# xyang9527/dro-sfm

Measured on AMD Instinct MI355X. Metric: training images/sec (KITTI 192x640 mf self-sup), higher is better.
Workload: dtype f32; 1 GPU; KITTI 192x640 mf self-sup (configs[1]); model=DepthPoseNet it8-seq4-inter-out, global_batch=2, per_gpu_batch=2, ref_frames=2, parallelism=dp1, optimizer=Adam lr 2e-4, execution=hipgraph, update_blocks=depth block + pose block (side stream, with both context encoders), encoder_3x3_s1=hip, encoder_strided=hip, exchange=none (world 1)

## Files before the change

dro-sfm_amd/csrc/conv.hip:

```cpp
#include <hip/hip_runtime.h>

#include <algorithm>
#include <cstddef>
#include <cstdio>
#include <cstdlib>
#include <cstring>
#include <map>
#include <mutex>
#include <string>
#include <type_traits>

#include "conv_common.hpp"
#include "dro_common.hpp"

namespace dro {


template <int BM, int MODE, int ACT, int EPI>
__global__ __launch_bounds__(256) void igemm_kernel(IgArgs a) {
  constexpr int WM = BM / 32;
  constexpr int KSTEPS = (WM == 2) ? 16 : 8;
  __shared__ float Ws[2][kBK][BM + 1];
  __shared__ float Xs[2][kBK][kBN];
  const int cb1 = a.cbase[1], cb2 = a.cbase[2], cb3 = a.cbase[3];
  const int H = a.g.H, W = a.g.W, KW = a.g.KW, PH = a.g.PH, PW = a.g.PW;
  const int Hsrc = a.Hs, Wsrc = a.Ws, sh = a.sshift;
  const unsigned HWs = (unsigned)Hsrc * (unsigned)Wsrc;
  const int Cin = a.g.Cin, Cout = a.g.Cout, rows = a.rows, kch = a.kch, K = a.K;
// ... 1025 lines not shown
  static constexpr int T = KH * KW;
  static constexpr bool TAPSPLIT = T == 9 && TG == 1;
  static constexpr int TPW = TAPSPLIT ? 5 : (TG == 3 ? 3 : T);
  static constexpr int TH = HaloShape<32, KH, KW>::TH, TW = 64 / TH;
  static constexpr int HWd = TW + KW - 1;
  static constexpr int HALO = (TH + KH - 1) * HWd;
  static constexpr int HPAD = HALO | 1;
  static constexpr int NJ = (HALO + 63) / 64;
  static constexpr int BC = 64, GPAD = 65;
  static constexpr int STAGE = 64 * GPAD + BC * HPAD;
  static constexpr int RED = TAPSPLIT ? 0 : 4 * 16 * 64;
  static constexpr int LDS = 2 * STAGE > RED ? 2 * STAGE : RED;
  static_assert(NJ <= 2 && TW % 2 == 0, "halo shape");
};

template <int KH, int KW, int GACT, bool MULTI, int TG>
__global__ __launch_bounds__(512) void wgrad2_kernel(typename WgParam<MULTI>::T P) {
  static_assert(TG == 1 || (TG == 3 && KH == 3 && KW == 3), "tap groups: 3x3 rows");
  const IgArgs& a = WgParam<MULTI>::ig(P);
  using S = HaloShapeW2<KH, KW, TG>;
  constexpr int T = S::T, TH = S::TH, TW = S::TW, HWd = S::HWd, HALO = S::HALO, HPAD = S::HPAD;
  constexpr int NJ = S::NJ, BC = S::BC, GPAD = S::GPAD, STAGE = S::STAGE, TPW = S::TPW;
  constexpr bool TAPSPLIT = S::TAPSPLIT;
  constexpr int PH = KH / 2, PW = KW / 2;
  __shared__ float smem[S::LDS];
  const int cb1 = a.cbase[1], cb2 = a.cbase[2], cb3 = a.cbase[3];
  const int H = a.g.H, W = a.g.W, Cin = a.g.Cin, Cout = a.g.Cout;
  const int tid = threadIdx.x, lane = tid & 63;
  const int wave = __builtin_amdgcn_readfirstlane(tid >> 6);
  const int noc = a.otiles * ((Cin + BC - 1) / BC);
  const int nbx = (int)gridDim.x;
  const int lin = xcd_remap((int)(blockIdx.x + blockIdx.y * gridDim.x), (int)(gridDim.x * gridDim.y));
  const int bx = lin % nbx, by = lin / nbx;
  const int tg = TG == 1 ? 0 : bx / noc;
  const int t = bx - tg * noc;
  const int ot = t % a.otiles, ct = t / a.otiles;
  const int o0 = ot * 64, c0 = ct * BC;
  const size_t HW = (size_t)H * W;
  const unsigned HWu = (unsigned)HW;
  int ntiles = a.g.B * a.tiles_img;
  if constexpr (MULTI) ntiles = P.use_tiles * P.nuse;
  const int tbeg = by * a.chunks_per_split;
  const int tend = min(ntiles, tbeg + a.chunks_per_split);
  const bool do_bias = a.gbias && ct == 0 && tg == 0;
  const float galpha = a.galpha;
  float gr[8], yr[GACT ? 8 : 1], xr[8 * NJ], bsum[8];
  unsigned gmask = 0, xmask = 0;
#pragma unroll
  for (int j = 0; j < 8; ++j) bsum[j] = 0.f;
  auto load = [&](int tile) {
    const float* __restrict__ Gp = a.G;
    const float* __restrict__ Yp = a.gy;
    KSlice sbase = kernarg_srcs();
    if constexpr (MULTI) {
      const int u = tile / P.use_tiles;
      tile -= u * P.use_tiles;
      Gp = *(KFPtr)(kernarg_base() + offsetof(WgMulti, uG) + u * sizeof(FPtr));
      if (GACT) Yp = *(KFPtr)(kernarg_base() + offsetof(WgMulti, uy) + u * sizeof(FPtr));
      sbase = (KSlice)(kernarg_base() + offsetof(WgMulti, usrc)) + u * kMaxSrc;
    }
    const int b = tile / a.tiles_img, trem = tile - b * a.tiles_img;
    const int ty0 = (trem / a.tiles_x) * TH, tx0 = (trem % a.tiles_x) * TW;
    const int qy = lane / TW, qx = lane - qy * TW;
    const int oy = ty0 + qy, ox = tx0 + qx;
    const bool pin = oy < H && ox < W;
    const unsigned pix = pin ? (unsigned)(oy * W + ox) : 0u;
    gmask = 0;
#pragma unroll
    for (int j = 0; j < 8; ++j) {
      const int o = o0 + wave * 8 + j;
      const bool ok = pin && o < Cout;
      gmask |= ok ? (1u << j) : 0u;
      const unsigned off = ok ? ((unsigned)b * Cout + o) * HWu + pix : 0u;
      gr[j] = Gp[off];
      if (GACT) yr[j] = Yp[off];
    }
    RowDesc ds[8];
// ... 37 lines not shown
        if (e < HPAD) Xs[(wave + 8 * i) * HPAD + e] = (xmask >> (i * NJ + j)) & 1u ? xr[i * NJ + j] : 0.f;
      }
    }
  };

  const int wo = wave & 1, wc = (wave >> 1) & 1, wg = wave >> 2;
  const int hi = lane >> 5;
  const int tap0 = TAPSPLIT ? wg * 5 : 0;
  const int ntap = TAPSPLIT ? (wg == 0 ? 5 : 4) : T;
  f32x16 acc[TPW];
#pragma unroll
  for (int tp = 0; tp < TPW; ++tp)
#pragma unroll
    for (int r = 0; r < 16; ++r) acc[tp][r] = 0.f;

  if (tbeg < tend) {
    load(tbeg);
    store(0);
  }
  __syncthreads();
  for (int tl = tbeg; tl < tend; ++tl) {
    const int buf = (tl - tbeg) & 1;
    const bool more = tl + 1 < tend;
    if (more) load(tl + 1);
    const float* Gs = smem + buf * STAGE;
    const float* Xs = Gs + 64 * GPAD;
    const float* ga = Gs + hi * GPAD + wo * 32 + (lane & 31);
    const float* xb = Xs + (wc * 32 + (lane & 31)) * HPAD + hi + (TG == 3 ? tg * HWd : 0);
    constexpr int KS = TAPSPLIT ? 32 : 16;
    const int pbase = TAPSPLIT ? 0 : wg * 16;
    auto kloop = [&](auto nt_c, int tbase) __attribute__((always_inline)) {
      constexpr int NT = decltype(nt_c)::value;
      int toff[NT];
#pragma unroll
      for (int k = 0; k < NT; ++k) {
        const int tap = tbase + k;
        toff[k] = (tap / KW) * HWd + (tap % KW);
      }
#pragma unroll 8
// ... 1 lines not shown
        const int pp = 2 * (pbase + s), poff = (pp / TW) * HWd + (pp % TW);
        const float av = ga[pp * GPAD];
#pragma unroll
        for (int k = 0; k < NT; ++k) acc[k] = mfma32(av, xb[poff + toff[k]], acc[k]);
      }
    };
    if constexpr (TAPSPLIT) {
      if (wg == 0) kloop(std::integral_constant<int, 5>{}, 0);
      else kloop(std::integral_constant<int, 4>{}, 5);
    } else {
      kloop(std::integral_constant<int, TPW>{}, 0);
    }
    if (more) store(buf ^ 1);
    __syncthreads();
  }
  float* wpart = a.part + (size_t)by * Cout * Cin * T;
  const int c = c0 + wc * 32 + (lane & 31);
  const size_t tstride = (size_t)Cout * Cin;
  if (TAPSPLIT) {
#pragma unroll
    for (int k = 0; k < TPW; ++k) {
      if (k < ntap) {
#pragma unroll
        for (int r = 0; r < 16; ++r) {
          const int o = o0 + wo * 32 + (r & 3) + 8 * (r >> 2) + 4 * (lane >> 5);
          if (o < Cout && c < Cin) wpart[(tap0 + k) * tstride + (size_t)o * Cin + c] = acc[k][r];
        }
      }
    }
  } else {
    float* red = smem;
// ... 9 lines not shown
#pragma unroll
        for (int r = 0; r < 16; ++r) {
          const int o = o0 + wo * 32 + (r & 3) + 8 * (r >> 2) + 4 * (lane >> 5);
          if (o < Cout && c < Cin)
            wpart[(tg * TPW + tp) * tstride + (size_t)o * Cin + c] = acc[tp][r] + red[(q4 * 16 + r) * 64 + lane];
        }
      }
      __syncthreads();
    }
  }
  if (do_bias) {
#pragma unroll
    for (int j = 0; j < 8; ++j) {
      const float v = wave_sum(bsum[j]);
      const int o = o0 + wave * 8 + j;
      if (lane == 0 && o < Cout) a.bpart[(size_t)by * Cout + o] = v;
    }
  }
}


template <int Q>
__global__ __launch_bounds__(256) void wgrad2_finish_kernel(IgArgs a, int splits) {
  constexpr int EPW = 64 / Q;
  const int Cout = a.g.Cout, Cin = a.g.Cin, T = a.g.KH * a.g.KW;
  const long long oc = (long long)Cout * Cin, total = oc * T;
  const int lane = threadIdx.x & 63, q = lane / EPW, le = lane - q * EPW;
  const int per = (splits + Q - 1) / Q;
  const int s0 = min(splits, q * per), n = min(splits, s0 + per) - s0;
  const long long wstride = (long long)gridDim.x * (blockDim.x / 64) * EPW;
  for (long long eb = ((long long)blockIdx.x * (blockDim.x / 64) + (threadIdx.x >> 6)) * EPW; eb < total;
       eb += wstride) {
    const long long e = eb + le;
    const bool ok = e < total;
    float v = ok ? split_sum(a.part + (size_t)s0 * total + e, (size_t)total, n) : 0.f;
    if (Q >= 4) v += __shfl_xor(v, 2 * EPW);
    if (Q >= 2) {
      const float o = __shfl_xor(v, EPW);
      v = q & 1 ? o + v : v + o;
    }
    if (ok && q == 0) {
      const int tap = (int)(e / oc);
      const long long r = e - (long long)tap * oc;
      const size_t dst = (size_t)r * T + tap;
      a.gweight[dst] = a.wacc ? a.gweight[dst] + v : v;
    }
  }
  if (a.gbias) {
    for (int e = blockIdx.x * blockDim.x + threadIdx.x; e < Cout; e += gridDim.x * blockDim.x) {
      const float bv = split_sum(a.bpart + e, (size_t)Cout, splits);
      a.gbias[e] = a.wacc ? a.gbias[e] + bv : bv;
    }
  }
}

static void launch_wgrad2_finish(const IgArgs& a, int splits, hipStream_t s) {
  const long long total = (long long)a.g.Cout * a.g.Cin * a.g.KH * a.g.KW;
  const int Q = splits >= 32 ? 4 : splits >= 8 ? 2 : 1;
  long long blocks = (total * Q + 255) / 256;
  if (blocks > 4096) blocks = 4096;
  if (Q == 4) hipLaunchKernelGGL(wgrad2_finish_kernel<4>, dim3((unsigned)blocks), dim3(256), 0, s, a, splits);
  else if (Q == 2) hipLaunchKernelGGL(wgrad2_finish_kernel<2>, dim3((unsigned)blocks), dim3(256), 0, s, a, splits);
  else hipLaunchKernelGGL(wgrad2_finish_kernel<1>, dim3((unsigned)blocks), dim3(256), 0, s, a, splits);
}

__global__ __launch_bounds__(256) void wgrad_halo_finish_kernel(IgArgs a, int splits) {
  const int Cout = a.g.Cout;
  const long long total = (long long)Cout * a.g.Cin * a.g.KH * a.g.KW;
// ... 2056 lines not shown
    else { DRO_WHM(3, 3); }
#undef DRO_WHM
  }
  if ((st = launch_status("wgrad_halo_kernel<multi> launch failed"))) return st;
  const long long total = (long long)Cout * Cin * T;
  long long blocks = (total + 255) / 256;
  if (blocks > 2048) blocks = 2048;
  if (v2)
    launch_wgrad2_finish(a, wh.splits, s);
  else
    hipLaunchKernelGGL(wgrad_halo_finish_kernel, dim3((unsigned)blocks), dim3(256), 0, s, a, wh.splits);
  return launch_status("wgrad_halo_finish_kernel launch failed");
}

namespace dro {
__global__ __launch_bounds__(256) void gru_elem_kernel(int stage, int hd, int HW,
                                                       const float* __restrict__ dhn,
                                                       const float* __restrict__ zr,
                                                       const float* __restrict__ q,
                                                       const float* __restrict__ h,
                                                       const float* __restrict__ drh,
                                                       float* __restrict__ dq,
                                                       float* __restrict__ dzr,
                                                       float* __restrict__ dh) {
  const int n = hd * HW;
  const int j = blockIdx.x * 256 + threadIdx.x;
  if (j >= n) return;
  const size_t b = blockIdx.y;
  const size_t i = b * n + j;
  const size_t zi = b * 2 * n + j, ri = zi + n;
// ... 35 lines not shown
```

dro-sfm_amd/hip/_lib.py:

```python
import ctypes
import os

import torch

_HERE = os.path.dirname(os.path.abspath(__file__))
LIB_PATH = os.environ.get("DRO_LIB_PATH") or os.path.normpath(os.path.join(_HERE, "..", "libdro_amd.so"))

_c_float_p = ctypes.c_void_p
_lib = None


def _sig(fn, *argtypes, restype=ctypes.c_int):
    fn.argtypes = list(argtypes)
    fn.restype = restype


def load():
    global _lib
    if _lib is not None:
        return _lib
    if not os.path.exists(LIB_PATH):
        raise RuntimeError(
            f"dro_sfm_amd: native library not found at {LIB_PATH}; build it with "
            "`make -C dro-sfm_amd/csrc` (or __graft_entry__.build()).  There is no CPU fallback.")
# ... 52 lines not shown
    _sig(lib.dro_batchnorm_relu_forward, P, P, P, P, I, I, I, I, F, F, P, P, P, P, P, P, P, Z, S)
    _sig(lib.dro_batchnorm_relu_backward, P, P, P, P, P, P, I, I, I, I, P, P, P, P, P, Z, S)
    _sig(lib.dro_conv2d_workspace_bytes, I, I, I, I, I, I, I, restype=Z)
    _sig(lib.dro_conv2d_plan, I, I, I, I, I, I, I, P)
    _sig(lib.dro_debug_conv_stamps, P)
    _sig(lib.dro_conv_log, I)
    _sig(lib.dro_conv_log_read, ctypes.c_char_p, ctypes.c_longlong, restype=ctypes.c_longlong)
    _sig(lib.dro_weight_split_bytes, I, I, I, I, I, restype=Z)
    _sig(lib.dro_weight_split, P, I, I, I, I, P, P, S)
    _sig(lib.dro_conv2d_forward, P, I, P, P, I, I, I, I, I, I, I, F, P, I, I, P, P, Z, S)
    _sig(lib.dro_convgru_gates_forward, P, I, P, P, I, I, I, I, I, I, P, P, P, P, Z, S)
    _sig(lib.dro_convgru_blend_forward, P, I, P, P, I, I, I, I, I, I, P, P, P, P, I, I, P, P, Z, S)
    _sig(lib.dro_conv2d_backward, P, I, P, I, I, I, I, I, I, I, F, P, P, P, P, P, P, P, P, I, P, P, Z, S)
    _sig(lib.dro_conv2d_weight_grad_multi_workspace_bytes, I, I, I, I, I, I, I, I, restype=Z)
    _sig(lib.dro_conv2d_weight_grad_multi, P, I, I, I, I, I, I, I, I, I, F, P, P, I, P, Z, S)
    _sig(lib.dro_adam_step, P, P, P, P, ctypes.c_longlong, P, P, S)
    _sig(lib.dro_gru_backward_elem, I, I, I, I, I, P, P, P, P, P, P, P, P, S)
    _sig(lib.dro_convgru_candidate_backward, P, I, P, I, I, I, I, I, I, P, P, P, P, P, P, P, P, P, P, Z, S)
    _sig(lib.dro_convgru_gates_backward, P, I, P, I, I, I, I, I, I, P, P, P, P, P, P, P, P, P, P, P, I, P, Z, S)
    _sig(lib.dro_bn_state_bytes, I, I, I, I, restype=Z)
    _sig(lib.dro_bn_apply, P, P, I, I, I, I, I, P, P, S)
    _sig(lib.dro_bn_backward_apply, P, P, I, I, I, I, P, P, S)
    _sig(lib.dro_conv2d_bn_forward, P, I, I, I, I, P, I, P, P, P, P, P, P, P, Z, S)
    _sig(lib.dro_conv2d_bn_backward_data, P, I, I, I, I, I, P, P, P, P, P, P, P, I, P, Z, S)
    _lib = lib
    return lib


EXPORTED = (
    "dro_last_error", "dro_abi_version", "dro_timestamp", "dro_wall_clock_hz",
# ... 7 lines not shown
    "dro_convex_upsample_many_backward",
    "dro_bilinear_upsample2x_forward", "dro_bilinear_upsample2x_backward",
    "dro_maxpool3x3s2_forward", "dro_maxpool3x3s2_backward",
    "dro_depth_metrics_blocks", "dro_depth_metrics_workspace_bytes", "dro_depth_metrics_prepare",
    "dro_depth_metrics_reduce", "dro_depth_metrics_median_workspace_bytes", "dro_depth_metrics_median",
    "dro_depth_metrics_demon_prepare", "dro_depth_metrics_demon_reduce",
    "dro_conv2d_strided_workspace_bytes", "dro_conv2d_strided_forward", "dro_conv2d_strided_backward",
    "dro_pose_mean_forward", "dro_pose_mean_backward",
    "dro_resize_rgb8_to_tensor", "dro_color_jitter_rgb8", "dro_resize_rgb8", "dro_rgb8_to_tensor",
    "dro_png_filtered_bytes", "dro_png_decode",
    "dro_batchnorm_workspace_bytes", "dro_batchnorm_relu_forward", "dro_batchnorm_relu_backward",
    "dro_weight_split_bytes", "dro_weight_split",
    "dro_conv2d_workspace_bytes", "dro_conv2d_plan", "dro_debug_conv_stamps", "dro_conv_log", "dro_conv_log_read", "dro_conv2d_forward", "dro_convgru_gates_forward",
    "dro_convgru_blend_forward", "dro_conv2d_backward",
    "dro_conv2d_weight_grad_multi_workspace_bytes", "dro_conv2d_weight_grad_multi",
    "dro_gru_backward_elem", "dro_convgru_candidate_backward", "dro_convgru_gates_backward", "dro_adam_step",
    "dro_bn_state_bytes", "dro_bn_apply", "dro_bn_backward_apply", "dro_conv2d_bn_forward", "dro_conv2d_bn_backward_data",
)


def check(status, what):
    if status != 0:
        msg = load().dro_last_error().decode(errors="replace")
        raise RuntimeError(f"{what} failed (status {status}): {msg}")


def ptr(t):
    return ctypes.c_void_p(t.data_ptr()) if t is not None else ctypes.c_void_p(0)


# ... 14 lines not shown
```

dro-sfm_amd/hip/conv.py:

```python
import contextlib
import ctypes
import os
from typing import Optional

import torch

from . import _lib
from ._lib import check, ptr, require_device, stream_of
from .ops import _sink_of

ACT = {None: 0, "none": 0, "relu": 1, "sigmoid": 2, "tanh": 3}


class DroSlice(ctypes.Structure):
    _fields_ = [("data", ctypes.c_void_p), ("channels", ctypes.c_int),
                ("total_channels", ctypes.c_int), ("channel_offset", ctypes.c_int),
                ("broadcast", ctypes.c_int)]


def _slice(t):
    B, C, H, W = t.shape
    s0, s1, s2, s3 = t.stride()
    if s2 == 0 and s3 == 0 and s1 == 1:
        return DroSlice(t.data_ptr(), C, s0 if B > 1 else C, 0, 1)
# ... 186 lines not shown
        ent = _PENDING[key] = ((B, H, W, Cin, Cout, KH, KW, act, float(alpha), gw, gb, len(srcs), weight), [], [])
    ent[1].append((list(srcs), dout, y))
    if all(s != cur for s in ent[2]):
        ent[2].append(cur)
    if not _PENDING_CB[0]:
        _PENDING_CB[0] = True
        stream = torch.cuda.current_stream()
        torch.autograd.Variable._execution_engine.queue_callback(lambda: flush_weight_grads(stream))
    return True


def _covers(t, ptr_):
    return t is not None and t.data_ptr() <= ptr_ < t.data_ptr() + t.numel() * t.element_size()


def flush_param_grads(param):
    g = param.grad
    if g is None or not _PENDING:
        return None
    p0 = g.data_ptr()
    keys = [k for k, (meta, _, _) in _PENDING.items() if _covers(meta[9], p0) or _covers(meta[10], p0)]
    if not keys:
        return None
    items = [_PENDING.pop(k) for k in keys]
    return _launch_weight_grads(items, items[0][2][0])


def flush_weight_grads(stream=None):
    _PENDING_CB[0] = False
    if not _PENDING:
        return
    items = list(_PENDING.values())
    _PENDING.clear()
    _launch_weight_grads(items, stream or torch.cuda.current_stream())


def _launch_weight_grads(items, stream):
    lib = _lib.load()
    side = any(s != stream for _, _, streams in items for s in streams)
    for _, uses, streams in items:
        for s in streams:
            if s != stream:
                stream.wait_stream(s)
    if side:
        for _, uses, streams in items:
            for srcs, dout, y in uses:
                for x in (*srcs, dout, y):
                    if x is not None:
                        x.record_stream(stream)
# ... 523 lines not shown
```

dro-sfm_amd/trainers/dp_trainer.py:

```python
import os
import sys
import time

import torch
import torch.distributed as dist


def graph_safe_nccl_env():
    os.environ.setdefault("TORCH_NCCL_TRACE_BUFFER_SIZE", "0")
    os.environ.setdefault("TORCH_NCCL_CUDA_EVENT_CACHE", "0")


_WATCHDOG_DRAIN_S = float(os.environ.get("DRO_WATCHDOG_DRAIN_S", "0.3"))


def drain_watchdog():
    if torch.cuda.is_available() and torch.cuda.is_initialized():
        torch.cuda.synchronize()
    time.sleep(_WATCHDOG_DRAIN_S)


def init_distributed(backend=None):
    graph_safe_nccl_env()
    world = int(os.environ.get("WORLD_SIZE", "1"))
# ... 12 lines not shown
    def __init__(self, params, bucket_mb=25.0, group=None, groups=(), direct_flush=None,
                 always_reduce=False):
        self.group = group
        self.world = dist.get_world_size(group) if dist.is_initialized() else 1
        self.reduce = self.world > 1 or (always_reduce and dist.is_initialized())
        self.suspend = False
        self.params = _adjacent_order([p for p in params if p.requires_grad], groups)
        if any(p.dtype != torch.float32 for p in self.params):
            raise RuntimeError("GradBuckets: fp32 parameters only")
        self.flat = torch.zeros(sum(p.numel() for p in self.params), device=self.params[0].device)
        self.offsets, off = {}, 0
        for p in self.params:
            self.offsets[p] = off
            p.grad = self.flat[off:off + p.numel()].view_as(p)
            off += p.numel()
        if direct_flush is None and self.flat.is_cuda:
            from ..hip.conv import flush_param_grads as direct_flush
        self.direct_flush = direct_flush
        self.bucket_bytes = int(bucket_mb * 1024 * 1024)
        self.active = None
        self.buckets, self._pending, self._seen = [], [], set()
        self.issued = []
        self.issued_in_backward = 0
        self.capture_origin = None
        self.issue_capturing = []
        self._hooks = [p.register_post_accumulate_grad_hook(self._on_grad) for p in self.params]
        self._comm = torch.cuda.Stream(device=self.flat.device) if self.flat.is_cuda else None
        for p in self.params:
            p._dro_direct = True

    def _build(self, active):
        self.active = [p for p in self.params if p in active]
# ... 29 lines not shown
        if direct and self.direct_flush is not None:
            wrote = self.direct_flush(p)
        if self.active is None:
            self._seen.add(p)
            return
        b = self._bucket_of.get(p)
        if b is None or self._ready[b]:
            return
        if self.flat.is_cuda:
            cur = torch.cuda.current_stream()
            self._bstreams[b].add(cur)
            if wrote is not None:
                (self._bstreams[b] if wrote == cur else self._bside[b]).add(wrote)
        self._left[b] -= 1
        if self._left[b] == 0:
            self._complete(b)
            self._issue_ready()

    def _complete(self, b):
        if self.flat.is_cuda:
            cur = torch.cuda.current_stream()
            for st in self._bstreams[b]:
                if st != cur:
                    cur.wait_stream(st)
        self._gather(b)
        if self.flat.is_cuda:
            self._events[b] = torch.cuda.Event()
            self._events[b].record(torch.cuda.current_stream())
        self._ready[b] = True

# ... 451 lines not shown
```

include/dro_amd.h:

```cpp
#ifndef DRO_AMD_H
#define DRO_AMD_H

#include <stddef.h>

#ifdef __cplusplus
extern "C" {
#endif

#define DRO_POSE_EULER 0
#define DRO_POSE_MATRIX 1

#define DRO_DEPTH_METRIC 0
#define DRO_DEPTH_INV 1
#define DRO_DEPTH_DISP 2

#define DRO_OK 0
#define DRO_E_NULL (-1)
#define DRO_E_SHAPE (-2)
#define DRO_E_MODE (-3)

const char* dro_last_error(void);
int dro_abi_version(void);

int dro_timestamp(unsigned long long* buf, int slot, void* stream);
// ... 209 lines not shown

typedef struct dro_wgrad_use {
  const dro_slice* srcs;
  const float* dout;
  const float* y;
} dro_wgrad_use;

size_t dro_conv2d_weight_grad_multi_workspace_bytes(int nuse, int B, int H, int W, int Cin, int Cout,
                                                    int KH, int KW);

int dro_conv2d_weight_grad_multi(const dro_wgrad_use* uses, int nuse, int nsrc, int B, int H, int W,
                                 int Cout, int KH, int KW, int act, float alpha, float* grad_weight,
                                 float* grad_bias, int accumulate, void* workspace,
                                 size_t workspace_bytes, void* stream);

int dro_gru_backward_elem(int stage, int B, int hd, int H, int W, const float* dhn,
                          const float* zr, const float* q, const float* h, const float* drh,
                          float* dq, float* dzr, float* dh, void* stream);

int dro_convgru_candidate_backward(const dro_slice* srcs, int nsrc, const float* weight, int B, int H, int W,
                                   int hd, int KH, int KW, const float* dq, const float* zr, const float* h,
                                   float* dzr, float* dh, float* const* grad_srcs, const int* grad_ctot,
                                   const int* grad_coff, const int* grad_accumulate, void* workspace,
                                   size_t workspace_bytes, void* stream);

int dro_convgru_gates_backward(const dro_slice* srcs, int nsrc, const float* weight, int B, int H, int W,
                               int hd, int KH, int KW, const float* dzr_in, float* const* grad_srcs,
                               const int* grad_ctot, const int* grad_coff, const int* grad_accumulate,
                               const float* prev_zr, const float* prev_q, const float* prev_h, float* prev_dq,
                               float* prev_dzr, float* prev_dh, int prev_dh_accumulate, void* workspace,
// ... 49 lines not shown
```

Baseline: 135.6 images/s.

## Group weight-gradient kernels of several conv layers into one launch

Adds a grouped weight-gradient path. Pending per-parameter weight-gradient jobs with the same kernel shape, activation and stream are batched, and up to eight layers are computed in a single wgrad2_group_kernel launch, followed by one grouped finish kernel. The per-block body is factored out so that blocks look up their member from a table in the kernel arguments. Tiles are strided across splits, and the DP trainer flushes ready groups when a gradient bucket completes. This is meant to cut launch count and fill the GPU better on small layers, at the cost of deferring some gradient work and adding host-side bookkeeping and a planner.

```diff
diff --git a/dro-sfm_amd/csrc/conv.hip b/dro-sfm_amd/csrc/conv.hip
--- a/dro-sfm_amd/csrc/conv.hip
+++ b/dro-sfm_amd/csrc/conv.hip
@@ -1,6 +1,7 @@
 #include <hip/hip_runtime.h>
 
 #include <algorithm>
+#include <climits>
 #include <cstddef>
 #include <cstdio>
 #include <cstdlib>
@@ -12,6 +13,7 @@
 
 #include "conv_common.hpp"
 #include "dro_common.hpp"
+#include "wgrad_group_plan.hpp"
 
 namespace dro {
 
@@ -1067,53 +1069,57 @@
   static_assert(NJ <= 2 && TW % 2 == 0, "halo shape");
 };
 
-template <int KH, int KW, int GACT, bool MULTI, int TG>
-__global__ __launch_bounds__(512) void wgrad2_kernel(typename WgParam<MULTI>::T P) {
+struct WgBlock {
+  int H, W, Cin, Cout, cb1, cb2, cb3;
+  int tiles_x, tiles_img, use_tiles;
+  int o0, c0, tg, tbeg, tend;
+  int tfirst, tstep;
+  bool do_bias;
+  float galpha;
+  float* wpart;
+  float* bpart;
+  const float* G;
+  const float* gy;
+  KSlice srcs;
+  unsigned uG, uy, usrc;
+};
+
+template <int KH, int KW, int GACT, bool TABLE, int TG>
+__device__ __forceinline__ void wgrad2_block(const WgBlock& k) {
   static_assert(TG == 1 || (TG == 3 && KH == 3 && KW == 3), "tap groups: 3x3 rows");
-  const IgArgs& a = WgParam<MULTI>::ig(P);
   using S = HaloShapeW2<KH, KW, TG>;
   constexpr int T = S::T, TH = S::TH, TW = S::TW, HWd = S::HWd, HALO = S::HALO, HPAD = S::HPAD;
-  constexpr int NJ = S::NJ, BC = S::BC, GPAD = S::GPAD, STAGE = S::STAGE, TPW = S::TPW;
+  constexpr int NJ = S::NJ, GPAD = S::GPAD, STAGE = S::STAGE, TPW = S::TPW;
   constexpr bool TAPSPLIT = S::TAPSPLIT;
   constexpr int PH = KH / 2, PW = KW / 2;
   __shared__ float smem[S::LDS];
-  const int cb1 = a.cbase[1], cb2 = a.cbase[2], cb3 = a.cbase[3];
-  const int H = a.g.H, W = a.g.W, Cin = a.g.Cin, Cout = a.g.Cout;
+  const int cb1 = k.cb1, cb2 = k.cb2, cb3 = k.cb3;
+  const int H = k.H, W = k.W, Cin = k.Cin, Cout = k.Cout;
   const int tid = threadIdx.x, lane = tid & 63;
   const int wave = __builtin_amdgcn_readfirstlane(tid >> 6);
-  const int noc = a.otiles * ((Cin + BC - 1) / BC);
-  const int nbx = (int)gridDim.x;
-  const int lin = xcd_remap((int)(blockIdx.x + blockIdx.y * gridDim.x), (int)(gridDim.x * gridDim.y));
-  const int bx = lin % nbx, by = lin / nbx;
-  const int tg = TG == 1 ? 0 : bx / noc;
-  const int t = bx - tg * noc;
-  const int ot = t % a.otiles, ct = t / a.otiles;
-  const int o0 = ot * 64, c0 = ct * BC;
+  const int tg = k.tg, o0 = k.o0, c0 = k.c0;
   const size_t HW = (size_t)H * W;
   const unsigned HWu = (unsigned)HW;
-  int ntiles = a.g.B * a.tiles_img;
-  if constexpr (MULTI) ntiles = P.use_tiles * P.nuse;
-  const int tbeg = by * a.chunks_per_split;
-  const int tend = min(ntiles, tbeg + a.chunks_per_split);
-  const bool do_bias = a.gbias && ct == 0 && tg == 0;
-  const float galpha = a.galpha;
+  const int tbeg = k.tbeg, tend = k.tend;
+  const bool do_bias = k.do_bias;
+  const float galpha = k.galpha;
   float gr[8], yr[GACT ? 8 : 1], xr[8 * NJ], bsum[8];
   unsigned gmask = 0, xmask = 0;
 #pragma unroll
   for (int j = 0; j < 8; ++j) bsum[j] = 0.f;
   auto load = [&](int tile) {
-    const float* __restrict__ Gp = a.G;
-    const float* __restrict__ Yp = a.gy;
-    KSlice sbase = kernarg_srcs();
-    if constexpr (MULTI) {
-      const int u = tile / P.use_tiles;
-      tile -= u * P.use_tiles;
-      Gp = *(KFPtr)(kernarg_base() + offsetof(WgMulti, uG) + u * sizeof(FPtr));
-      if (GACT) Yp = *(KFPtr)(kernarg_base() + offsetof(WgMulti, uy) + u * sizeof(FPtr));
-      sbase = (KSlice)(kernarg_base() + offsetof(WgMulti, usrc)) + u * kMaxSrc;
-    }
-    const int b = tile / a.tiles_img, trem = tile - b * a.tiles_img;
-    const int ty0 = (trem / a.tiles_x) * TH, tx0 = (trem % a.tiles_x) * TW;
+    const float* __restrict__ Gp = k.G;
+    const float* __restrict__ Yp = k.gy;
+    KSlice sbase = k.srcs;
+    if constexpr (TABLE) {
+      const int u = tile / k.use_tiles;
+      tile -= u * k.use_tiles;
+      Gp = *(KFPtr)(kernarg_base() + k.uG + u * sizeof(FPtr));
+      if (GACT) Yp = *(KFPtr)(kernarg_base() + k.uy + u * sizeof(FPtr));
+      sbase = (KSlice)(kernarg_base() + k.usrc) + u * kMaxSrc;
+    }
+    const int b = tile / k.tiles_img, trem = tile - b * k.tiles_img;
+    const int ty0 = (trem / k.tiles_x) * TH, tx0 = (trem % k.tiles_x) * TW;
     const int qy = lane / TW, qx = lane - qy * TW;
     const int oy = ty0 + qy, ox = tx0 + qx;
     const bool pin = oy < H && ox < W;
@@ -1181,15 +1187,16 @@
 #pragma unroll
     for (int r = 0; r < 16; ++r) acc[tp][r] = 0.f;
 
+  const int tfirst = k.tfirst, tstep = k.tstep;
   if (tbeg < tend) {
-    load(tbeg);
+    load(tfirst + tbeg * tstep);
     store(0);
   }
   __syncthreads();
   for (int tl = tbeg; tl < tend; ++tl) {
     const int buf = (tl - tbeg) & 1;
     const bool more = tl + 1 < tend;
-    if (more) load(tl + 1);
+    if (more) load(tfirst + (tl + 1) * tstep);
     const float* Gs = smem + buf * STAGE;
     const float* Xs = Gs + 64 * GPAD;
     const float* ga = Gs + hi * GPAD + wo * 32 + (lane & 31);
@@ -1221,7 +1228,7 @@
     if (more) store(buf ^ 1);
     __syncthreads();
   }
-  float* wpart = a.part + (size_t)by * Cout * Cin * T;
+  float* wpart = k.wpart;
   const int c = c0 + wc * 32 + (lane & 31);
   const size_t tstride = (size_t)Cout * Cin;
   if (TAPSPLIT) {
@@ -1261,22 +1268,134 @@
     for (int j = 0; j < 8; ++j) {
       const float v = wave_sum(bsum[j]);
       const int o = o0 + wave * 8 + j;
-      if (lane == 0 && o < Cout) a.bpart[(size_t)by * Cout + o] = v;
-    }
-  }
-}
-
+      if (lane == 0 && o < Cout) k.bpart[o] = v;
+    }
+  }
+}
+
+template <int KH, int KW, int GACT, bool MULTI, int TG>
+__global__ __launch_bounds__(512) void wgrad2_kernel(typename WgParam<MULTI>::T P) {
+  const IgArgs& a = WgParam<MULTI>::ig(P);
+  constexpr int BC = HaloShapeW2<KH, KW, TG>::BC, T = KH * KW;
+  const int Cin = a.g.Cin, Cout = a.g.Cout;
+  const int noc = a.otiles * ((Cin + BC - 1) / BC);
+  const int nbx = (int)gridDim.x;
+  const int lin = xcd_remap((int)(blockIdx.x + blockIdx.y * gridDim.x), (int)(gridDim.x * gridDim.y));
+  const int bx = lin % nbx, by = lin / nbx;
+  const int tg = TG == 1 ? 0 : bx / noc;
+  const int t = bx - tg * noc;
+  const int ot = t % a.otiles, ct = t / a.otiles;
+  int ntiles = a.g.B * a.tiles_img;
+  if constexpr (MULTI) ntiles = P.use_tiles * P.nuse;
+  WgBlock k;
+  k.H = a.g.H, k.W = a.g.W, k.Cin = Cin, k.Cout = Cout;
+  k.cb1 = a.cbase[1], k.cb2 = a.cbase[2], k.cb3 = a.cbase[3];
+  k.tiles_x = a.tiles_x, k.tiles_img = a.tiles_img, k.use_tiles = 0;
+  k.o0 = ot * 64, k.c0 = ct * BC, k.tg = tg;
+  k.tbeg = by * a.chunks_per_split;
+  k.tend = min(ntiles, k.tbeg + a.chunks_per_split);
+  k.tfirst = 0, k.tstep = 1;
+  k.do_bias = a.gbias && ct == 0 && tg == 0;
+  k.galpha = a.galpha;
+  k.wpart = a.part + (size_t)by * Cout * Cin * T;
+  k.bpart = a.bpart + (size_t)by * Cout;
+  k.G = a.G, k.gy = a.gy, k.srcs = kernarg_srcs();
+  k.uG = k.uy = k.usrc = 0;
+  if constexpr (MULTI) {
+    k.use_tiles = P.use_tiles;
+    k.uG = offsetof(WgMulti, uG), k.uy = offsetof(WgMulti, uy), k.usrc = offsetof(WgMulti, usrc);
+  }
+  wgrad2_block<KH, KW, GACT, MULTI, TG>(k);
+}
+
+struct WgGroupMember {
+  int H, W, Cin, Cout, cb1, cb2, cb3;
+  int tiles_x, tiles_img, use_tiles, ntiles;
+  int otiles, noc, splits;
+  int use0;
+  int block0, fin0, fin_blocks;
+  int finish_q, wacc;
+  float galpha;
+  float* part;
+  float* bpart;
+  float* gweight;
+  float* gbias;
+};
+
+struct WgGroupHead {
+  int T;
+  int block0[kGroupMembers];
+  int fin0[kGroupMembers];
+  WgGroupMember m[kGroupMembers];
+};
+
+struct WgGroup {
+  WgGroupHead h;
+  Slice usrc[kGroupUses][kMaxSrc];
+  const float* uG[kGroupUses];
+  const float* uy[kGroupUses];
+};
+static_assert(sizeof(WgGroup) <= 4096, "grouped weight gradient: kernel arguments over 4 KiB");
+
+typedef __attribute__((address_space(4))) const WgGroupMember* KMember;
+
+__device__ __forceinline__ int group_member_of(const int (&first)[kGroupMembers], int id) {
+  int mi = 0;
+#pragma unroll
+  for (int i = 1; i < kGroupMembers; ++i) mi += id >= first[i] ? 1 : 0;
+  return mi;
+}
+
+template <int KH, int KW, int GACT>
+__global__ __launch_bounds__(512) void wgrad2_group_kernel(WgGroup P) {
+  constexpr int T = KH * KW;
+  const int lin = xcd_remap((int)blockIdx.x, (int)gridDim.x);
+  const int mi = group_member_of(P.h.block0, lin);
+  const KMember km = (KMember)(kernarg_base() + offsetof(WgGroup, h) + offsetof(WgGroupHead, m)) + mi;
+  const int local = lin - km->block0;
+  const int noc = km->noc, otiles = km->otiles;
+  const int by = local / noc, t = local - by * noc;
+  const int ot = t % otiles, ct = t / otiles;
+  const int Cin = km->Cin, Cout = km->Cout, use0 = km->use0;
+  WgBlock k;
+  k.H = km->H, k.W = km->W, k.Cin = Cin, k.Cout = Cout;
+  k.cb1 = km->cb1, k.cb2 = km->cb2, k.cb3 = km->cb3;
+  k.tiles_x = km->tiles_x, k.tiles_img = km->tiles_img, k.use_tiles = km->use_tiles;
+  k.o0 = ot * 64, k.c0 = ct * 64, k.tg = 0;
+  const int splits = km->splits, ntiles = km->ntiles;
+  k.tbeg = 0;
+  k.tend = (ntiles - by + splits - 1) / splits;
+  k.tfirst = by, k.tstep = splits;
+  k.do_bias = km->gbias && ct == 0;
+  k.galpha = km->galpha;
+  k.wpart = km->part + (size_t)by * Cout * Cin * T;
+  k.bpart = km->bpart + (size_t)by * Cout;
+  k.G = nullptr, k.gy = nullptr, k.srcs = kernarg_srcs();
+  k.uG = (unsigned)(offsetof(WgGroup, uG) + use0 * sizeof(FPtr));
+  k.uy = (unsigned)(offsetof(WgGroup, uy) + use0 * sizeof(FPtr));
+  k.usrc = (unsigned)(offsetof(WgGroup, usrc) + use0 * kMaxSrc * sizeof(Slice));
+  wgrad2_block<KH, KW, GACT, true, 1>(k);
+}
+
+
+struct WgFinish {
+  const float* part;
+  const float* bpart;
+  float* gweight;
+  float* gbias;
+  int wacc, Cout, Cin, T, splits, block, nblocks;
+};
 
 template <int Q>
-__global__ __launch_bounds__(256) void wgrad2_finish_kernel(IgArgs a, int splits) {
+__device__ __forceinline__ void wgrad2_finish_block(const WgFinish& a) {
   constexpr int EPW = 64 / Q;
-  const int Cout = a.g.Cout, Cin = a.g.Cin, T = a.g.KH * a.g.KW;
+  const int Cout = a.Cout, Cin = a.Cin, T = a.T, splits = a.splits;
   const long long oc = (long long)Cout * Cin, total = oc * T;
   const int lane = threadIdx.x & 63, q = lane / EPW, le = lane - q * EPW;
   const int per = (splits + Q - 1) / Q;
   const int s0 = min(splits, q * per), n = min(splits, s0 + per) - s0;
-  const long long wstride = (long long)gridDim.x * (blockDim.x / 64) * EPW;
-  for (long long eb = ((long long)blockIdx.x * (blockDim.x / 64) + (threadIdx.x >> 6)) * EPW; eb < total;
+  const long long wstride = (long long)a.nblocks * (blockDim.x / 64) * EPW;
+  for (long long eb = ((long long)a.block * (blockDim.x / 64) + (threadIdx.x >> 6)) * EPW; eb < total;
        eb += wstride) {
     const long long e = eb + le;
     const bool ok = e < total;
@@ -1294,11 +1413,34 @@
     }
   }
   if (a.gbias) {
-    for (int e = blockIdx.x * blockDim.x + threadIdx.x; e < Cout; e += gridDim.x * blockDim.x) {
+    for (int e = a.block * blockDim.x + threadIdx.x; e < Cout; e += a.nblocks * blockDim.x) {
       const float bv = split_sum(a.bpart + e, (size_t)Cout, splits);
       a.gbias[e] = a.wacc ? a.gbias[e] + bv : bv;
     }
   }
+}
+
+template <int Q>
+__global__ __launch_bounds__(256) void wgrad2_finish_kernel(IgArgs a, int splits) {
+  WgFinish f;
+  f.part = a.part, f.bpart = a.bpart, f.gweight = a.gweight, f.gbias = a.gbias, f.wacc = a.wacc;
+  f.Cout = a.g.Cout, f.Cin = a.g.Cin, f.T = a.g.KH * a.g.KW, f.splits = splits;
+  f.block = (int)blockIdx.x, f.nblocks = (int)gridDim.x;
+  wgrad2_finish_block<Q>(f);
+}
+
+__global__ __launch_bounds__(256) void wgrad2_group_finish_kernel(WgGroupHead P) {
+  const int id = (int)blockIdx.x;
+  const int mi = group_member_of(P.fin0, id);
+  const KMember km = (KMember)(kernarg_base() + offsetof(WgGroupHead, m)) + mi;
+  WgFinish f;
+  f.part = km->part, f.bpart = km->bpart, f.gweight = km->gweight, f.gbias = km->gbias, f.wacc = km->wacc;
+  f.Cout = km->Cout, f.Cin = km->Cin, f.T = P.T, f.splits = km->splits;
+  f.block = id - km->fin0, f.nblocks = km->fin_blocks;
+  const int Q = km->finish_q;
+  if (Q == 4) wgrad2_finish_block<4>(f);
+  else if (Q == 2) wgrad2_finish_block<2>(f);
+  else wgrad2_finish_block<1>(f);
 }
 
 static void launch_wgrad2_finish(const IgArgs& a, int splits, hipStream_t s) {
@@ -3385,6 +3527,142 @@
 }
 
 namespace dro {
+namespace {
+
+int group_setup(const dro_wgrad_member* members, int nmember, int KH, int KW, int act, WgGroupPlan* pl,
+                WgGroup* g) {
+  if (!members) {
+    set_error("conv2d_weight_grad_group: NULL members");
+    return DRO_E_NULL;
+  }
+  if (nmember < 1 || nmember > kGroupMembers) {
+    set_error("conv2d_weight_grad_group: need 1..8 members per call (dro_conv2d_weight_grad_group_capacity)");
+    return DRO_E_SHAPE;
+  }
+  if (!wgrad_group_shape_ok(KH, KW)) {
+    set_error("conv2d_weight_grad_group: kernel shape not supported (1x1, 1x5, 5x1, 3x3)");
+    return DRO_E_SHAPE;
+  }
+  if (act < 0 || act > 3) {
+    set_error("conv2d_weight_grad_group: unknown activation");
+    return DRO_E_MODE;
+  }
+  WgGroupShape shapes[kGroupMembers];
+  int nuse = 0, st;
+  for (int i = 0; i < nmember; ++i) {
+    const dro_wgrad_member& mb = members[i];
+    if (!mb.uses || !mb.grad_weight) {
+      set_error("conv2d_weight_grad_group: NULL uses/grad_weight");
+      return DRO_E_NULL;
+    }
+    if (mb.nuse < 1 || mb.nuse > kGroupUsesPerMember) {
+      set_error("conv2d_weight_grad_group: need 1..16 uses per member");
+      return DRO_E_SHAPE;
+    }
+    if (nuse + mb.nuse > kGroupUses) {
+      set_error("conv2d_weight_grad_group: more uses than use slots (dro_conv2d_weight_grad_group_capacity)");
+      return DRO_E_SHAPE;
+    }
+    IgArgs first = {};
+    for (int u = 0; u < mb.nuse; ++u) {
+      IgArgs t = {};
+      if ((st = conv_setup_geom(t, mb.uses[u].srcs, mb.nsrc, mb.B, mb.H, mb.W, mb.Cout, KH, KW))) return st;
+      if (!mb.uses[u].dout || (act != 0 && !mb.uses[u].y)) {
+        set_error("conv2d_weight_grad_group: NULL dout (or y with an activation)");
+        return DRO_E_NULL;
+      }
+      if (u == 0) first = t;
+      for (int j = 0; j < kMaxSrc; ++j)
+        if (t.cbase[j] != first.cbase[j]) {
+          set_error("conv2d_weight_grad_group: uses split the input channels differently");
+          return DRO_E_SHAPE;
+        }
+      if (g) {
+        for (int j = 0; j < kMaxSrc; ++j) g->usrc[nuse + u][j] = t.src[j];
+        g->uG[nuse + u] = mb.uses[u].dout;
+        g->uy[nuse + u] = act ? mb.uses[u].y : nullptr;
+      }
+    }
+    shapes[i] = {mb.nuse, mb.B, mb.H, mb.W, first.g.Cin, mb.Cout};
+    if (g) {
+      WgGroupMember& m = g->h.m[i];
+      m.H = mb.H, m.W = mb.W, m.Cin = first.g.Cin, m.Cout = mb.Cout;
+      m.cb1 = first.cbase[1], m.cb2 = first.cbase[2], m.cb3 = first.cbase[3];
+      m.galpha = mb.alpha;
+      m.gweight = mb.grad_weight;
+      m.gbias = mb.grad_bias;
+      m.wacc = mb.accumulate ? 1 : 0;
+    }
+    nuse += mb.nuse;
+  }
+  static const int target = [] {
+    const int v = env_int("DRO_WGG_TARGET_BLOCKS", 0);
+    return v > 0 ? v : kGroupTarget;
+  }();
+  if (!wgrad_group_plan(shapes, nmember, KH, KW, target, pl)) {
+    set_error("conv2d_weight_grad_group: the group cannot be planned");
+    return DRO_E_SHAPE;
+  }
+  return DRO_OK;
+}
+
+}
+}
+
+extern "C" int dro_conv2d_weight_grad_group_capacity(int* max_members, int* max_uses) {
+  if (max_members) *max_members = kGroupMembers;
+  if (max_uses) *max_uses = kGroupUses;
+  return (int)sizeof(WgGroup);
+}
+
+extern "C" size_t dro_conv2d_weight_grad_group_workspace_bytes(const dro_wgrad_member* members, int nmember,
+                                                              int KH, int KW) {
+  WgGroupPlan pl;
+  return group_setup(members, nmember, KH, KW, 0, &pl, nullptr) == DRO_OK ? pl.bytes : 0;
+}
+
+extern "C" int dro_conv2d_weight_grad_group(const dro_wgrad_member* members, int nmember, int KH, int KW,
+                                            int act, void* workspace, size_t workspace_bytes, void* stream) {
+  WgGroup g = {};
+  WgGroupPlan pl;
+  int st;
+  if ((st = group_setup(members, nmember, KH, KW, act, &pl, &g))) return st;
+  if ((st = check_ws(workspace, workspace_bytes, pl.bytes, "conv2d_weight_grad_group"))) return st;
+  char* ws = static_cast<char*>(workspace);
+  const int T = KH * KW;
+  double flops = 0.0;
+  g.h.T = T;
+  for (int i = 0; i < kGroupMembers; ++i) g.h.block0[i] = g.h.fin0[i] = INT_MAX;
+  for (int i = 0; i < nmember; ++i) {
+    const WgGroupMemberPlan& p = pl.m[i];
+    WgGroupMember& m = g.h.m[i];
+    m.tiles_x = p.tiles_x, m.tiles_img = p.tiles_img, m.use_tiles = p.use_tiles, m.ntiles = p.ntiles;
+    m.otiles = p.otiles, m.noc = p.otiles * p.ctiles;
+    m.splits = p.splits;
+    m.use0 = p.use0;
+    m.block0 = g.h.block0[i] = p.block0;
+    m.fin0 = g.h.fin0[i] = p.fin0;
+    m.fin_blocks = p.fin_blocks;
+    m.finish_q = p.finish_q;
+    m.part = reinterpret_cast<float*>(ws + p.part_off);
+    m.bpart = reinterpret_cast<float*>(ws + p.bpart_off);
+    flops += 2.0 * m.Cout * m.Cin * T * (double)members[i].B * m.H * m.W * members[i].nuse;
+  }
+  hipStream_t s = (hipStream_t)stream;
+  const dim3 grid((unsigned)pl.blocks);
+  conv_logf(flops, "wgrad2_group_kernel<%d, %d, %d>", KH, KW, act);
+#define DRO_WGG(KH_, KW_) DRO_ACT_SWITCH(act, hipLaunchKernelGGL((wgrad2_group_kernel<KH_, KW_, A_>), grid, dim3(512), 0, s, g))
+  if (KH == 1 && KW == 1) { DRO_WGG(1, 1); }
+  else if (KH == 1) { DRO_WGG(1, 5); }
+  else if (KW == 1) { DRO_WGG(5, 1); }
+  else { DRO_WGG(3, 3); }
+#undef DRO_WGG
+  if ((st = launch_status("wgrad2_group_kernel launch failed"))) return st;
+  hipLaunchKernelGGL(wgrad2_group_finish_kernel, dim3((unsigned)pl.fin_blocks), dim3(256), 0, s, g.h);
+  return launch_status("wgrad2_group_finish_kernel launch failed");
+}
+
+namespace dro {
 __global__ __launch_bounds__(256) void gru_elem_kernel(int stage, int hd, int HW,
                                                        const float* __restrict__ dhn,
                                                        const float* __restrict__ zr,
diff --git a/dro-sfm_amd/csrc/wgrad_group_plan.hpp b/dro-sfm_amd/csrc/wgrad_group_plan.hpp
--- /dev/null
+++ b/dro-sfm_amd/csrc/wgrad_group_plan.hpp
@@ -0,0 +1,104 @@
+#pragma once
+#include <cstddef>
+
+namespace dro {
+
+constexpr int kGroupMembers = 8;
+constexpr int kGroupUses = 24;
+constexpr int kGroupUsesPerMember = 16;
+constexpr int kGroupTarget = 256;
+constexpr int kGroupMaxSplits = 256;
+
+struct WgGroupShape {
+  int nuse, B, H, W, Cin, Cout;
+};
+
+struct WgGroupMemberPlan {
+  int tiles_x, tiles_img;
+  int use_tiles, ntiles;
+  int otiles, ctiles;
+  int tiles_per_split, splits;
+  int block0, blocks;
+  int finish_q;
+  int fin0, fin_blocks;
+  int use0;
+  size_t part_off, bpart_off;
+};
+
+struct WgGroupPlan {
+  int nmember, blocks, fin_blocks, nuse;
+  size_t bytes;
+  WgGroupMemberPlan m[kGroupMembers];
+};
+
+inline bool wgrad_group_shape_ok(int KH, int KW) {
+  return (KH == 1 && KW == 5) || (KH == 5 && KW == 1) || (KH == 3 && KW == 3) || (KH == 1 && KW == 1);
+}
+
+inline size_t wgrad_group_align(size_t n) { return (n + 255) & ~(size_t)255; }
+
+inline bool wgrad_group_plan(const WgGroupShape* s, int n, int KH, int KW, int target, WgGroupPlan* pl) {
+  if (!s || !pl || n < 1 || n > kGroupMembers || !wgrad_group_shape_ok(KH, KW) || target < 1) return false;
+  const int TH = (KW == 1 || (KH == 3 && KW == 3)) ? 8 : 4, TW = 64 / TH, T = KH * KW;
+  long long work = 0;
+  int nuse = 0;
+  for (int i = 0; i < n; ++i) {
+    if (s[i].nuse < 1 || s[i].nuse > kGroupUsesPerMember || s[i].B < 1 || s[i].H < 1 || s[i].W < 1 ||
+        s[i].Cin < 1 || s[i].Cout < 1)
+      return false;
+    WgGroupMemberPlan& m = pl->m[i];
+    m.tiles_x = (s[i].W + TW - 1) / TW;
+    m.tiles_img = ((s[i].H + TH - 1) / TH) * m.tiles_x;
+    m.use_tiles = s[i].B * m.tiles_img;
+    m.ntiles = s[i].nuse * m.use_tiles;
+    m.otiles = (s[i].Cout + 63) / 64;
+    m.ctiles = (s[i].Cin + 63) / 64;
+    m.use0 = nuse;
+    nuse += s[i].nuse;
+    work += (long long)m.ntiles * m.otiles * m.ctiles;
+  }
+  if (nuse > kGroupUses) return false;
+  long long tps = (work + target - 1) / target, max_tiles = 1;
+  for (int i = 0; i < n; ++i) max_tiles = pl->m[i].ntiles > max_tiles ? pl->m[i].ntiles : max_tiles;
+  auto blocks_at = [&](long long t) {
+    long long b = 0;
+    for (int i = 0; i < n; ++i) {
+      long long sp = (pl->m[i].ntiles + t - 1) / t;
+      b += (long long)pl->m[i].otiles * pl->m[i].ctiles * (sp > kGroupMaxSplits ? kGroupMaxSplits : sp);
+    }
+    return b;
+  };
+  if (blocks_at(max_tiles) > target) tps = max_tiles;
+  while (tps < max_tiles && blocks_at(tps) > target) ++tps;
+  int block = 0, fin = 0;
+  size_t off = 0;
+  for (int i = 0; i < n; ++i) {
+    WgGroupMemberPlan& m = pl->m[i];
+    long long sp = (m.ntiles + tps - 1) / tps;
+    if (sp > kGroupMaxSplits) sp = kGroupMaxSplits;
+    m.tiles_per_split = (int)((m.ntiles + sp - 1) / sp);
+    m.splits = (m.ntiles + m.tiles_per_split - 1) / m.tiles_per_split;
+    m.block0 = block;
+    m.blocks = m.otiles * m.ctiles * m.splits;
+    block += m.blocks;
+    m.finish_q = m.splits >= 32 ? 4 : m.splits >= 8 ? 2 : 1;
+    const long long total = (long long)s[i].Cout * s[i].Cin * T;
+    long long fb = (total * m.finish_q + 255) / 256;
+    if (fb > 4096) fb = 4096;
+    m.fin0 = fin;
+    m.fin_blocks = (int)fb;
+    fin += m.fin_blocks;
+    m.part_off = off;
+    off += wgrad_group_align((size_t)m.splits * (size_t)total * sizeof(float));
+    m.bpart_off = off;
+    off += wgrad_group_align((size_t)m.splits * s[i].Cout * sizeof(float));
+  }
+  pl->nmember = n;
+  pl->blocks = block;
+  pl->fin_blocks = fin;
+  pl->nuse = nuse;
+  pl->bytes = off;
+  return true;
+}
+
+}
diff --git a/dro-sfm_amd/hip/_lib.py b/dro-sfm_amd/hip/_lib.py
--- a/dro-sfm_amd/hip/_lib.py
+++ b/dro-sfm_amd/hip/_lib.py
@@ -90,6 +90,9 @@
     _sig(lib.dro_conv2d_backward, P, I, P, I, I, I, I, I, I, I, F, P, P, P, P, P, P, P, P, I, P, P, Z, S)
     _sig(lib.dro_conv2d_weight_grad_multi_workspace_bytes, I, I, I, I, I, I, I, I, restype=Z)
     _sig(lib.dro_conv2d_weight_grad_multi, P, I, I, I, I, I, I, I, I, I, F, P, P, I, P, Z, S)
+    _sig(lib.dro_conv2d_weight_grad_group_capacity, P, P)
+    _sig(lib.dro_conv2d_weight_grad_group_workspace_bytes, P, I, I, I, restype=Z)
+    _sig(lib.dro_conv2d_weight_grad_group, P, I, I, I, I, P, Z, S)
     _sig(lib.dro_adam_step, P, P, P, P, ctypes.c_longlong, P, P, S)
     _sig(lib.dro_gru_backward_elem, I, I, I, I, I, P, P, P, P, P, P, P, P, S)
     _sig(lib.dro_convgru_candidate_backward, P, I, P, I, I, I, I, I, I, P, P, P, P, P, P, P, P, P, P, Z, S)
@@ -127,6 +130,8 @@
     "dro_conv2d_workspace_bytes", "dro_conv2d_plan", "dro_debug_conv_stamps", "dro_conv_log", "dro_conv_log_read", "dro_conv2d_forward", "dro_convgru_gates_forward",
     "dro_convgru_blend_forward", "dro_conv2d_backward",
     "dro_conv2d_weight_grad_multi_workspace_bytes", "dro_conv2d_weight_grad_multi",
+    "dro_conv2d_weight_grad_group_capacity", "dro_conv2d_weight_grad_group_workspace_bytes",
+    "dro_conv2d_weight_grad_group",
     "dro_gru_backward_elem", "dro_convgru_candidate_backward", "dro_convgru_gates_backward", "dro_adam_step",
     "dro_bn_state_bytes", "dro_bn_apply", "dro_bn_backward_apply", "dro_conv2d_bn_forward", "dro_conv2d_bn_backward_data",
 )
diff --git a/dro-sfm_amd/hip/conv.py b/dro-sfm_amd/hip/conv.py
--- a/dro-sfm_amd/hip/conv.py
+++ b/dro-sfm_amd/hip/conv.py
@@ -224,6 +224,53 @@
     return t is not None and t.data_ptr() <= ptr_ < t.data_ptr() + t.numel() * t.element_size()
 
 
+class DroWgradMember(ctypes.Structure):
+    _fields_ = [("uses", ctypes.c_void_p), ("nuse", ctypes.c_int), ("nsrc", ctypes.c_int),
+                ("B", ctypes.c_int), ("H", ctypes.c_int), ("W", ctypes.c_int), ("Cout", ctypes.c_int),
+                ("alpha", ctypes.c_float), ("grad_weight", ctypes.c_void_p), ("grad_bias", ctypes.c_void_p),
+                ("accumulate", ctypes.c_int)]
+
+
+_GROUPED = [os.environ.get("DRO_GROUPED_WGRAD", "1") != "0"]
+_READY = {}
+_GROUP_CAP = []
+GROUP_LAUNCHES = []
+GROUP_LOG = [False]
+
+
+def set_grouped_weight_grads(enabled):
+    _GROUPED[0] = bool(enabled)
+
+
+def _group_capacity():
+    if not _GROUP_CAP:
+        m, u = ctypes.c_int(0), ctypes.c_int(0)
+        _lib.load().dro_conv2d_weight_grad_group_capacity(ctypes.byref(m), ctypes.byref(u))
+        _GROUP_CAP[:] = [m.value, u.value]
+    return _GROUP_CAP
+
+
+def _groupable(item):
+    meta, uses, streams = item
+    return (_GROUPED[0] and (meta[5], meta[6]) in _MULTI_SHAPES and len(streams) == 1
+            and len(uses) <= _MAX_USES)
+
+
+def _ready(item):
+    meta, uses, streams = item
+    key = (streams[0], meta[5], meta[6], meta[7])
+    group = _READY.setdefault(key, [])
+    max_members, max_uses = _group_capacity()
+    if (len(group) + 1 > max_members or sum(len(it[1]) for it in group) + len(uses) > max_uses
+            or any(it[0][9].data_ptr() == meta[9].data_ptr() for it in group)):
+        _launch_group(key, _READY.pop(key))
+        group = _READY.setdefault(key, [])
+    group.append(item)
+    if len(group) == max_members or sum(len(it[1]) for it in group) == max_uses:
+        _launch_group(key, _READY.pop(key))
+    return streams[0]
+
+
 def flush_param_grads(param):
     g = param.grad
     if g is None or not _PENDING:
@@ -233,16 +280,70 @@
     if not keys:
         return None
     items = [_PENDING.pop(k) for k in keys]
-    return _launch_weight_grads(items, items[0][2][0])
+    stream = items[0][2][0]
+    single = [it for it in items if not _groupable(it)]
+    for it in items:
+        if _groupable(it):
+            _ready(it)
+    if single:
+        _launch_weight_grads(single, stream)
+    return stream
+
+
+def flush_ready_groups(lo=None, hi=None):
+    streams = set()
+    for key in list(_READY):
+        group = _READY[key]
+        if lo is None or any(lo <= t.data_ptr() < hi for it in group for t in it[0][9:11] if t is not None):
+            _launch_group(key, _READY.pop(key))
+            streams.add(key[0])
+    return streams
 
 
 def flush_weight_grads(stream=None):
     _PENDING_CB[0] = False
-    if not _PENDING:
-        return
     items = list(_PENDING.values())
     _PENDING.clear()
-    _launch_weight_grads(items, stream or torch.cuda.current_stream())
+    single = [it for it in items if not _groupable(it)]
+    for it in items:
+        if _groupable(it):
+            _ready(it)
+    cur = torch.cuda.current_stream()
+    for s in flush_ready_groups():
+        if s != cur:
+            cur.wait_stream(s)
+    if single:
+        _launch_weight_grads(single, stream or cur)
+
+
+def _launch_group(key, group):
+    if not group:
+        return
+    lib = _lib.load()
+    stream, KH, KW, act = key
+    n = len(group)
+    keep, members = [], (DroWgradMember * n)()
+    for i, (meta, uses, _) in enumerate(group):
+        B, H, W, Cin, Cout, _, _, _, alpha, gw, gb, nsrc, _ = meta
+        sl = [_slices(srcs) for srcs, _, _ in uses]
+        arr = (DroWgradUse * len(uses))()
+        for j, (_, dout, y) in enumerate(uses):
+            arr[j].srcs = ctypes.cast(sl[j], ctypes.c_void_p)
+            arr[j].dout = dout.data_ptr()
+            arr[j].y = y.data_ptr() if y is not None else None
+        keep.append((sl, arr))
+        m = members[i]
+        m.uses, m.nuse, m.nsrc = ctypes.cast(arr, ctypes.c_void_p), len(uses), nsrc
+        m.B, m.H, m.W, m.Cout, m.alpha = B, H, W, Cout, alpha
+        m.grad_weight, m.grad_bias, m.accumulate = gw.data_ptr(), gb.data_ptr() if gb is not None else None, 1
+    if GROUP_LOG[0]:
+        GROUP_LAUNCHES.append((KH, KW, act, [(len(u), *m[:5]) for m, u, _ in group]))
+    with torch.cuda.stream(stream):
+        nb = int(lib.dro_conv2d_weight_grad_group_workspace_bytes(members, n, KH, KW))
+        ws = torch.empty(max(nb, 1), dtype=torch.uint8, device=group[0][0][9].device)
+        check(lib.dro_conv2d_weight_grad_group(members, n, KH, KW, act, ptr(ws), nb,
+                                               ctypes.c_void_p(stream.cuda_stream)),
+              "dro_conv2d_weight_grad_group")
 
 
 def _launch_weight_grads(items, stream):
diff --git a/dro-sfm_amd/trainers/dp_trainer.py b/dro-sfm_amd/trainers/dp_trainer.py
--- a/dro-sfm_amd/trainers/dp_trainer.py
+++ b/dro-sfm_amd/trainers/dp_trainer.py
@@ -50,8 +50,10 @@
             self.offsets[p] = off
             p.grad = self.flat[off:off + p.numel()].view_as(p)
             off += p.numel()
+        self.bucket_flush = None
         if direct_flush is None and self.flat.is_cuda:
-            from ..hip.conv import flush_param_grads as direct_flush
+            from ..hip.conv import flush_param_grads as direct_flush, flush_ready_groups
+            self.bucket_flush = flush_ready_groups
         self.direct_flush = direct_flush
         self.bucket_bytes = int(bucket_mb * 1024 * 1024)
         self.active = None
@@ -111,6 +113,9 @@
                 (self._bstreams[b] if wrote == cur else self._bside[b]).add(wrote)
         self._left[b] -= 1
         if self._left[b] == 0:
+            if self.reduce and self.bucket_flush is not None:
+                sl = self._slice(self.buckets[b])
+                self.bucket_flush(sl.data_ptr(), sl.data_ptr() + sl.numel() * sl.element_size())
             self._complete(b)
             self._issue_ready()
 
diff --git a/include/dro_amd.h b/include/dro_amd.h
--- a/include/dro_amd.h
+++ b/include/dro_amd.h
@@ -247,6 +247,25 @@
                                  float* grad_bias, int accumulate, void* workspace,
                                  size_t workspace_bytes, void* stream);
 
+typedef struct dro_wgrad_member {
+  const dro_wgrad_use* uses;
+  int nuse;
+  int nsrc;
+  int B, H, W, Cout;
+  float alpha;
+  float* grad_weight;
+  float* grad_bias;
+  int accumulate;
+} dro_wgrad_member;
+
+int dro_conv2d_weight_grad_group_capacity(int* max_members, int* max_uses);
+
+size_t dro_conv2d_weight_grad_group_workspace_bytes(const dro_wgrad_member* members, int nmember,
+                                                    int KH, int KW);
+
+int dro_conv2d_weight_grad_group(const dro_wgrad_member* members, int nmember, int KH, int KW,
+                                 int act, void* workspace, size_t workspace_bytes, void* stream);
+
 int dro_gru_backward_elem(int stage, int B, int hd, int H, int W, const float* dhn,
                           const float* zr, const float* q, const float* h, const float* drh,
                           float* dq, float* dzr, float* dh, void* stream);
```

Result: faster. 141.8 images/s, median of 6 (+4.6%).
